# hahnyuan/PTQ4ViT

Hardware: AMD Instinct MI355X
Metric: calibration throughput (wrapped modules calibrated per second), ViT-B/224 W8A8, 32 calibration images (higher is better)
Workload: dtype int8

## Files before the change

### include/ptq4vit_hip_debug.h

```cpp
#ifndef PTQ4VIT_HIP_DEBUG_H
#define PTQ4VIT_HIP_DEBUG_H

#include <stdint.h>

#ifdef __cplusplus
extern "C" {
#endif

int p4v_debug_set_variant(int variant, int force_generic);
int p4v_debug_set_tuning(int key, int value);
int p4v_debug_topk_rows(const float* d_mass, int segs, int n, int k, int32_t* d_idx, void* stream);
int p4v_debug_pack_dual(const float* d_x, long rows, long cols, long cols_padded, int sos, int lo, int hi, int qmax,
                        const float* d_scale, float const_scale, int8_t* d_q1, int8_t* d_q2, void* stream);
int p4v_debug_pack_cands(const float* d_x, long rows, long cols, long rows_padded, long cols_padded, int layout, int lo, int hi,
                         const float* d_scales, int n_cands, const int* d_crange, const unsigned char* d_done, int live_max,
                         int general, int8_t* d_q, void* stream);
int p4v_debug_gather_im2col(int batch, int in_channels, int height, int width, int kernel_h, int kernel_w, int stride_h, int stride_w,
                            int pad_h, int pad_w, int dil_h, int dil_w, const float* d_x, const int32_t* d_idx, int k, float* d_dst,
                            void* stream);
int p4v_debug_prep_epi6(const float* d_o, const float* d_wt, const float* d_bias, long o_ss, long o_ts, int sr, int tr,
                        int bias_on_t, int wt_mode, int transposed, float* d_e, void* stream);

#ifdef __cplusplus
}
#endif
#endif
```

### ptq4vit_amd/_lib.py

```python
import ctypes as C
import os

_HERE = os.path.dirname(os.path.abspath(__file__))
LIB_PATH = os.environ.get("P4V_LIB") or os.path.join(_HERE, "csrc", "libptq4vit_hip.so")

METRICS = {
    "L1_norm": 0,
    "L2_norm": 1,
    "linear_weighted_L2_norm": 2,
    "square_weighted_L2_norm": 3,
    "hessian": 4,
    "cosine": 5,
}


class LinearDesc(C.Structure):
    _fields_ = [(n, C.c_int32) for n in (
        "batch", "tokens", "in_features", "out_features", "n_V", "n_H", "n_a", "w_bit", "a_bit", "metric",
        "eq_n", "search_round", "twin_postgelu", "init_layerwise", "has_bias", "reserved")]


class MatMulDesc(C.Structure):
    _fields_ = ([(n, C.c_int32) for n in ("batch", "heads", "M", "K", "N")] + [("_pad0", C.c_int32)] +
                [("a_stride", C.c_int64 * 4), ("b_stride", C.c_int64 * 4)] +
# ... 10 lines not shown
        "batch", "in_channels", "height", "width", "out_channels", "kernel_h", "kernel_w", "stride_h", "stride_w",
        "pad_h", "pad_w", "dil_h", "dil_w", "w_bit", "a_bit", "metric", "eq_n", "search_round", "channelwise",
        "init_layerwise", "has_bias", "reserved")]


class KernelStats(C.Structure):
    _fields_ = [("sweep_i8_ms", C.c_double), ("sweep_i8_launches", C.c_int64), ("sweep_i8_macs", C.c_double),
                ("sweep_f32_ms", C.c_double), ("sweep_f32_launches", C.c_int64), ("sweep_f32_macs", C.c_double),
                ("sweep_i8_alg_macs", C.c_double), ("sweep_f32_alg_macs", C.c_double),
                ("sweep6_ms", C.c_double), ("sweep6_launches", C.c_int64), ("sweep6_macs", C.c_double), ("sweep6_alg_macs", C.c_double),
                ("memo_hits", C.c_int64), ("memo_misses", C.c_int64),
                ("sweep7_ms", C.c_double), ("sweep7_launches", C.c_int64), ("sweep7_macs", C.c_double), ("sweep7_alg_macs", C.c_double),
                ("sweep7_twin_ms", C.c_double), ("sweep7_twin_launches", C.c_int64), ("event_overhead_ms", C.c_double)]


class LaunchRecord(C.Structure):
    _fields_ = [("kind", C.c_int32), ("stage", C.c_int32), ("grid_x", C.c_int32), ("grid_z", C.c_int32),
                ("ms", C.c_double), ("ops", C.c_double), ("alg_ops", C.c_double), ("alg_bytes", C.c_double)]


LAUNCH_KINDS = {0: "k_sweep<int8>", 1: "k_sweep<float>", 2: "k_sweep6", 3: "k_sweep7", 4: "k_sweep7 (twin)", 5: "k_sweep4/5", 6: "k_sweep9",
                7: "k_sweep8", 8: "k_sweep2g", 9: "k_sweep2", 11: "k_sos_split", 12: "k_bound", 13: "k_slice_b", 14: "k_slice_a", 15: "k_sweep_seg"}
LAUNCH_STAGES = {0: "full", 1: "A", 2: "B1", 3: "B2", 4: "A2"}


class PlaneDesc(C.Structure):
    _fields_ = [("rows", C.c_int64), ("cols", C.c_int64), ("cols_padded", C.c_int64), ("rows_per_scale", C.c_int64),
                ("mode", C.c_int32), ("lo", C.c_int32), ("hi", C.c_int32), ("qmax", C.c_int32),
                ("const_scale", C.c_float), ("reserved", C.c_int32)]


class ExportDesc(C.Structure):
    _fields_ = [("dims", C.c_int32 * 4), ("src_stride", C.c_int64 * 4),
                ("scale1_stride", C.c_int64 * 4), ("scale1_div", C.c_int32 * 4),
                ("scale2_stride", C.c_int64 * 4), ("scale2_div", C.c_int32 * 4),
                ("scale2_const", C.c_float),
                ("mode", C.c_int32), ("lo1", C.c_int32), ("hi1", C.c_int32), ("lo2", C.c_int32), ("hi2", C.c_int32),
                ("qmax", C.c_int32), ("reserved", C.c_int32)]


class GroupJob(C.Structure):
    _fields_ = [("kind", C.c_int32), ("status", C.c_int32), ("desc", C.c_void_p), ("inp", C.c_void_p * 5), ("mult", C.c_void_p),
                ("out", C.c_void_p * 3), ("workspace", C.c_void_p), ("workspace_bytes", C.c_size_t)]


JOB_LINEAR, JOB_MATMUL, JOB_CONV, JOB_MATMUL_BLOCKS = 0, 1, 2, 3
PLANE_SYM, PLANE_SOS_HI, PLANE_SOS_LO, PLANE_TWIN = 1, 2, 3, 4
EXPORT_SYM_I8, EXPORT_SYM_F32, EXPORT_GELU_U8, EXPORT_SOS_U8 = 0, 1, 2, 3


EXPORTS = [
    "p4v_version", "p4v_last_error",
    "p4v_linear_workspace_bytes", "p4v_linear_calibrate",
    "p4v_matmul_workspace_bytes", "p4v_matmul_calibrate",
    "p4v_matmul_blocks_workspace_bytes", "p4v_matmul_blocks_calibrate", "p4v_amax_init_matmul_blocks",
    "p4v_matmul_blocks_search", "p4v_matmul_blocks_quant_forward",
    "p4v_conv_workspace_bytes", "p4v_conv_calibrate",
    "p4v_calibrate_group", "p4v_launch_counters",
    "p4v_linear_quant_forward", "p4v_matmul_quant_forward",
    "p4v_amax_init_linear", "p4v_linear_search_w", "p4v_linear_search_a",
    "p4v_amax_init_matmul", "p4v_matmul_search_A", "p4v_sos_search_split", "p4v_matmul_search_B",
    "p4v_amax_init_conv", "p4v_conv_search_w_channelwise", "p4v_conv_search_w_layerwise", "p4v_conv_search_a",
    "p4v_score_argmax_gather",
    "p4v_quantize_i8", "p4v_pack_plane_i8", "p4v_fake_quant", "p4v_export_quantize", "p4v_multi_copy",
    "p4v_stats_enable", "p4v_stats_reset", "p4v_stats_get", "p4v_stats_launches", "p4v_prune_counters",
    "p4v_debug_set_variant", "p4v_debug_set_tuning", "p4v_debug_topk_rows", "p4v_debug_pack_dual", "p4v_debug_prep_epi6",
    "p4v_debug_pack_cands", "p4v_debug_gather_im2col",
]

_lib = None


def load():
    global _lib
    if _lib is not None:
        return _lib
    if not os.path.exists(LIB_PATH):
        raise RuntimeError(
            f"ptq4vit_amd: HIP extension {LIB_PATH} is missing -- build it with "
            "`python -c 'import __graft_entry__ as g; g.build()'` (hipcc --offload-arch=gfx950). "
            "There is no CPU fallback for the calibration path.")
    import torch
    lib = C.CDLL(LIB_PATH)
    vp, fp, ip = C.c_void_p, C.c_void_p, C.c_void_p
    lib.p4v_version.restype = C.c_int
    lib.p4v_last_error.restype = C.c_char_p
    lib.p4v_linear_workspace_bytes.restype = C.c_size_t
    lib.p4v_linear_workspace_bytes.argtypes = [C.POINTER(LinearDesc)]
    lib.p4v_linear_calibrate.restype = C.c_int
    lib.p4v_linear_calibrate.argtypes = [C.POINTER(LinearDesc), fp, fp, fp, fp, fp, fp, fp, fp, fp, ip, vp, C.c_size_t, vp]
# ... 38 lines not shown
        fn.restype = C.c_int
        fn.argtypes = args + tail
    lib.p4v_score_argmax_gather.restype = C.c_int
    lib.p4v_score_argmax_gather.argtypes = [fp, C.c_int32, C.c_int32, fp, fp, ip, vp]
    lib.p4v_quantize_i8.restype = C.c_int
    lib.p4v_quantize_i8.argtypes = [fp, C.c_int64, C.c_int64, C.c_int64, fp, C.c_int64, C.c_int32, C.c_int32, vp, vp]
    lib.p4v_fake_quant.restype = C.c_int
    lib.p4v_fake_quant.argtypes = [fp, C.c_int64, C.c_int64, fp, C.c_int64, C.c_int32, C.c_int32, fp, vp]
    lib.p4v_pack_plane_i8.restype = C.c_int
    lib.p4v_pack_plane_i8.argtypes = [C.POINTER(PlaneDesc), fp, fp, vp, vp]
    lib.p4v_export_quantize.restype = C.c_int
    lib.p4v_export_quantize.argtypes = [C.POINTER(ExportDesc), fp, fp, fp, vp, vp]
    lib.p4v_multi_copy.restype = C.c_int
    lib.p4v_multi_copy.argtypes = [vp, C.c_int32, C.c_int64, C.c_int64, vp]
    lib.p4v_debug_topk_rows.restype = C.c_int
    lib.p4v_debug_topk_rows.argtypes = [vp, C.c_int, C.c_int, C.c_int, vp, vp]
    lib.p4v_debug_pack_dual.restype = C.c_int
    lib.p4v_debug_pack_dual.argtypes = [fp, C.c_long, C.c_long, C.c_long, C.c_int, C.c_int, C.c_int, C.c_int, fp, C.c_float, vp, vp, vp]
    lib.p4v_debug_pack_cands.restype = C.c_int
    lib.p4v_debug_pack_cands.argtypes = [fp, C.c_long, C.c_long, C.c_long, C.c_long, C.c_int, C.c_int, C.c_int, fp, C.c_int, vp, vp,
                                         C.c_int, C.c_int, vp, vp]
    lib.p4v_debug_gather_im2col.restype = C.c_int
    lib.p4v_debug_gather_im2col.argtypes = [C.c_int] * 12 + [fp, ip, C.c_int, fp, vp]
    lib.p4v_debug_prep_epi6.restype = C.c_int
    lib.p4v_debug_prep_epi6.argtypes = [fp, fp, fp, C.c_long, C.c_long, C.c_int, C.c_int, C.c_int, C.c_int, C.c_int, fp, vp]
    lib.p4v_debug_set_variant.restype = C.c_int
    lib.p4v_debug_set_variant.argtypes = [C.c_int, C.c_int]
    lib.p4v_debug_set_tuning.restype = C.c_int
    lib.p4v_debug_set_tuning.argtypes = [C.c_int, C.c_int]
    lib.p4v_stats_enable.restype = C.c_int
    lib.p4v_stats_enable.argtypes = [C.c_int]
    lib.p4v_stats_reset.restype = C.c_int
    lib.p4v_stats_get.restype = C.c_int
    lib.p4v_stats_get.argtypes = [C.POINTER(KernelStats)]
    lib.p4v_stats_launches.restype = C.c_int
    lib.p4v_stats_launches.argtypes = [C.POINTER(LaunchRecord), C.c_int64, C.POINTER(C.c_int64)]
    lib.p4v_prune_counters.restype = C.c_int
    lib.p4v_prune_counters.argtypes = [C.POINTER(C.c_int64), C.c_int]
    lib.p4v_launch_counters.restype = C.c_int
    lib.p4v_launch_counters.argtypes = [C.POINTER(C.c_int64), C.c_int]
    lib.p4v_calibrate_group.restype = C.c_int
    lib.p4v_calibrate_group.argtypes = [C.POINTER(GroupJob), C.c_int32, vp, vp]
    _lib = lib
    return lib


# ... 17 lines not shown
```

### ptq4vit_amd/csrc/p4v_api.hip

```cpp
#include <hip/hip_runtime.h>

#include <algorithm>
#include <atomic>
#include <climits>
#include <cstdarg>
#include <cstdio>
#include <condition_variable>
#include <cstring>
#include <deque>
#include <functional>
#include <thread>
#include <mutex>
#include <string>
#include <unordered_map>
#include <type_traits>
#include <vector>

#include "../../include/ptq4vit_hip.h"
#include "../../include/ptq4vit_hip_debug.h"
#include "p4v_kernels.h"

using namespace p4v;

namespace {
// ... 43 lines not shown
        return (dry || top > cap) ? nullptr : base + cap - top;
    }
    bool ok() const { return dry || off + top <= cap; }
};

struct StatRec { hipEvent_t a, b; int kind; double macs, alg; int stage, gx, gz; double ms, bytes; };
thread_local double g_alg_bytes = 0;
thread_local double g_alg_macs_cand = 0;
thread_local double g_exec_frac = 1.0;
thread_local bool g_stat_on = false;
thread_local std::vector<StatRec> g_stat_recs;
thread_local std::vector<StatRec> g_stat_done;
thread_local int g_stage = 0;
thread_local p4v_kernel_stats g_stats = {};
thread_local long g_memo_hits = 0, g_memo_misses = 0;
std::atomic<long long> g_prune_cnt[4];
constexpr int VARIANT_KEPT = 1 | 2 | 4 | 2048 | 32768 | 65536 | 131072 | 524288 | 1048576 | 2097152 | 4194304 | 8388608 | 134217728;
std::atomic<int> g_variant_word{0};
#define g_variant (g_variant_word.load(std::memory_order_relaxed) & 0x3fffffff)
#define g_force_v1 ((g_variant_word.load(std::memory_order_relaxed) >> 30) & 1)
std::atomic<int> g_tune[16];
enum { TUNE_CG6 = 0, TUNE_CG2 = 1, TUNE_CG2G = 2, TUNE_CG7 = 3, TUNE_PRINT = 4, TUNE_ORDER7 = 5, TUNE_P6 = 6, TUNE_PLANE_GIB = 7, TUNE_EPI6W = 8,
       TUNE_LOOSE_PCT = 9, TUNE_SLICE_DIV = 10, TUNE_SLICE_SMALL = 11, TUNE_B1_PATH = 12, TUNE_TIER2 = 13, TUNE_TIER2_DIV = 14, TUNE_LOOSE_ROWS = 15 };
inline bool tune_b1_removed(int v) { return v == 1 || v == 2 || v == 3 || v == 5 || v == 6 || v == 8 || v == 10 || v == 12; }
inline int tune(int k) { return g_tune[k].load(std::memory_order_relaxed); }

struct Group;
struct Ctx {
    hipStream_t st;
    Arena ws;
    bool dry;
    Group* grp = nullptr;
    int slot = 0;
    int par = 1;
};

struct StatInfo { int kind; double macs, alg; int stage, gx, gz; double bytes; };
struct QOp;
struct KernelDesc {
    hipError_t (*one)(const QOp&, hipStream_t);
    hipError_t (*many)(const QOp* const*, int, hipStream_t);
    int cap;
};
constexpr int QOP_PARAM_BYTES = 480;
struct QOp {
    enum Type : int { KERNEL, FILL, D2H, H2D, COPY2D, WAIT };
    int type = KERNEL;
// ... 73 lines not shown
    int n = 0;
    std::mutex mu;
    std::condition_variable cv;
    std::vector<std::deque<QOp>> q;
    std::vector<int> state;
    int blocked = 0;
    unsigned long gen = 0;
    int status = 0;
    std::string err;
    std::vector<int*> mirrors;
    bool stat_on = false;
    std::vector<StatRec>* stat_recs = nullptr;
    long n_ops = 0, n_launches = 0, n_rounds = 0;
    hipEvent_t inputs_ready = nullptr;
    bool waited = false;
    int last_par[16] = {};
    int issue_kernels(std::vector<const QOp*>& ops);
    int issue_round();
    int sync(int slot);
    void finish(int slot);
};

std::atomic<long long> g_launch_cnt[4];
int enqueue_now(hipStream_t st, const QOp& op, bool timed, std::vector<StatRec>* recs) {
    g_launch_cnt[1].fetch_add(1, std::memory_order_relaxed);
    StatRec rec{};
    if (timed) {
        HIPCHK(hipEventCreate(&rec.a));
        HIPCHK(hipEventCreate(&rec.b));
        HIPCHK(hipEventRecord(rec.a, st));
    }
    HIPCHK(op.kd->one(op, st));
    if (timed) {
        HIPCHK(hipEventRecord(rec.b, st));
        rec.kind = op.si.kind; rec.macs = op.si.macs; rec.alg = op.si.alg; rec.stage = op.si.stage; rec.gx = op.si.gx; rec.gz = op.si.gz; rec.bytes = op.si.bytes;
        recs->push_back(rec);
    }
    return 0;
}
int issue_plain(hipStream_t st, const QOp& op) {
    switch (op.type) {
        case QOp::FILL: HIPCHK(hipMemsetAsync(op.dst, op.value, op.bytes, st)); break;
        case QOp::D2H: HIPCHK(hipMemcpyAsync(op.dst, op.src, op.bytes, hipMemcpyDeviceToHost, st)); break;
        case QOp::H2D: HIPCHK(hipMemcpyAsync(op.dst, op.payload.data(), op.bytes, hipMemcpyHostToDevice, st)); break;
        case QOp::COPY2D: HIPCHK(hipMemcpy2DAsync(op.dst, op.dpitch, op.src, op.spitch, op.width, op.height, hipMemcpyDeviceToDevice, st)); break;
        default: break;
// ... 491 lines not shown
    cgroups = std::max(cgroups, cdiv(nc, per_max));
    const int per = cdiv(nc, cgroups);
    const size_t lds = (size_t)SW7_NS * SW7_STAGE + (size_t)per * 192 + 256;
    Sweep7Params q = p;
    q.cgroups = cgroups;
    dim3 grid(p.rtiles * p.ctiles * cgroups, 1, 1);
    const StatInfo si = stat_info(twin ? 4 : 3, (double)p.rtiles * 256 * (double)p.ctiles * 256 * (double)p.ldk * nc, g_alg_macs_cand * nc,
                                  (int)grid.x, (int)grid.z, g_alg_bytes);
    const StatInfo* sp = &si;
    return twin == 2 ? launch_sweep7_epi<2>(c, q, epi, grid, lds, sp) : twin ? launch_sweep7_epi<1>(c, q, epi, grid, lds, sp) : launch_sweep7_epi<0>(c, q, epi, grid, lds, sp);
}

int launch_sweep(Ctx& c, const SweepParams& p, bool i8, bool twin, int epi, bool fast = false, int cgroups = 1) {
    if (c.dry) return 0;
    const int kind = (fast && p.bound) ? 12 : (fast && p.halves > 0) ? 6 : (fast && sweep8_ok(p, twin, epi)) ? 7 :
                     (fast && epi != EPI_COS && sweep2g_ok(p)) ? 8 : fast ? 9 : i8 ? 0 : 1;
    const double kelems = (double)p.ldk / (i8 ? 1 : 4);
    const StatInfo si = stat_info(kind, (double)p.mtiles * SW_BM * (double)p.ntiles * SW_BN * kelems * p.Z * (p.c1 - p.c0) * (twin ? 2 : 1),
                                  g_alg_macs_cand * (p.c1 - p.c0),
                                  (fast && p.bound) ? p.mtiles * p.ntiles * 2 : (fast && p.halves > 0) ? p.halves : p.mtiles * p.ntiles, cgroups, g_alg_bytes);
    const StatInfo* sp = &si;
    if (fast && p.bound) {
        const dim3 grid(p.mtiles * p.ntiles * 2), block(256);
        P4V_EPI4(epi, return enqueue(c, KERN_T(SweepParams, k_bound, E), grid, block, 0, p, sp))
    }
    if (fast && p.halves > 0) return p.a_cs == 0 ? launch_sweep9_epi<true>(c, p, epi, cgroups, sp) : launch_sweep9_epi<false>(c, p, epi, cgroups, sp);
    if (fast && sweep8_ok(p, twin, epi)) return p.a_cs == 0 ? launch_sweep8_epi<true>(c, p, epi, cgroups, sp) : launch_sweep8_epi<false>(c, p, epi, cgroups, sp);
    if (fast && epi != EPI_COS && sweep2g_ok(p)) return twin ? launch_sweep2g_epi<true>(c, p, epi, cgroups, sp) : launch_sweep2g_epi<false>(c, p, epi, cgroups, sp);
    if (fast) return twin ? launch_sweep2_epi<true>(c, p, epi, cgroups, sp) : launch_sweep2_epi<false>(c, p, epi, cgroups, sp);
    if (i8) return twin ? launch_sweep_epi<int8_t, true>(c, p, epi, cgroups, sp) : launch_sweep_epi<int8_t, false>(c, p, epi, cgroups, sp);
    return twin ? launch_sweep_epi<float, true>(c, p, epi, cgroups, sp) : launch_sweep_epi<float, false>(c, p, epi, cgroups, sp);
}

int launch_finish(Ctx& c, const FinishParams& p) {
    return enqueue(c, KERN(FinishParams, k_finish), dim3(p.C, p.nj), dim3(256), 0, p);
}

int launch_finish_cos(Ctx& c, const FinishCosParams& p) {
    const int gy = p.j_mode == 3 ? cdiv(p.S, 256) : p.nj;
    return enqueue(c, KERN(FinishCosParams, k_finish_cos), dim3(p.C, gy), dim3(p.j_mode == 3 ? 256 : 1024), 0, p);
}

int launch_select(Ctx& c, const SelectParams& p_) {
    if (c.dry) return 0;
    SelectParams p = p_;
    attach_mirror(p);
    return enqueue(c, KERN(SelectParams, k_select), dim3(p.nj), dim3(128), 0, p);
// ... 496 lines not shown
        sp.ldk = Kp * esz; sp.ktiles = sp.ldk / SW_BKB;
        sp.S1 = S1; sp.S2 = S2; sp.s_cs = ps.s_cs; sp.sb_mode = ps.sb_mode; sp.sb_div = std::max(1, ps.sb_div);
        sp.bias = ps.bias; sp.bias_axis = ps.bias_axis; sp.bias_zs = ps.bias_zs;
        sp.O = ps.O; sp.Wt = ps.G ? ps.G : ps.O; sp.wt_mode = ps.wt_mode;
        sp.o_zs = ps.o_zs; sp.o_bs = ps.o_bs; sp.o_ms = ps.o_ms; sp.o_nbs = ps.o_nbs; sp.o_ns = ps.o_ns;
        sp.o_inner = ps.o_inner > 0 ? ps.o_inner : INT_MAX;
        sp.o_ninner = ps.o_ninner > 0 ? ps.o_ninner : INT_MAX;
        sp.M = ps.Mrows; sp.N = ps.Ncols; sp.Z = ps.Z; sp.c0 = c0; sp.c1 = c0 + nc; sp.crange = ps.crange;
        sp.crange_blk = rblk_z; sp.cb_div = std::max(1, ps.j_div);
        sp.part = part; sp.p_cs = p_cs; sp.p_zs = p_zs; sp.Np = NpP;
        sp.mtiles = Mp / SW_BM; sp.ntiles = Np / SW_BN;
        sp.dbg = g_variant & 3;
        sp.store = ps.store_out;
        int cgroups = 1;
        if (!fast && !fast_cos) {
            const long wgs = (long)sp.mtiles * sp.ntiles * ps.Z;
            cgroups = choose_cgroups(wgs, nc, sp.ktiles, cu_slots(c, 512, ps.i8 ? 0 : 1), 20.0, ps.i8 ? 1.6 : 2.6);
        }
        if (fast || fast_cos) {
            const long wgs = (long)sp.mtiles * sp.ntiles * ps.Z;
            cgroups = choose_cgroups(wgs, nc, sp.ktiles, cu_slots(c, ps.twin ? 256 : 512, 9), ps.twin ? 40.0 : 25.0, ps.twin ? 0.45 : 0.40);
        }
        sp.bound = bound ? 1 : 0;
        if (bound) sp.dbg = tune(TUNE_B1_PATH) >= 16 ? (tune(TUNE_B1_PATH) >> 4) : 0;
        if (bound) { sp.A = rowbuf; sp.B = colbuf; sp.a_cs = sp.b_cs = 0; }
        if (fast && !bound && !ps.store_out && (ps.j_mode == 0 || ps.j_mode == 2)) {
            const int h9 = sweep9_halves(sp, ps.twin, ps.epi);
            if (h9 > 0 && (long)h9 * SW9_NW <= p_zs) {
                sp.halves = h9;
                sp.rows_p_stream = sp.a_cs == 0 ? Np : Mp;
                sp.p_zs = (long)h9 * SW9_NW; sp.p_cs = sp.p_zs * ps.Z;
                nine_halves = h9;
                cgroups = choose_cgroups((long)h9 * ps.Z, nc, 1, cu_slots(c, SW9_NW == 4 ? 512 : 256, 6), 12.0, 0.9);
            }
        }
        if (fast && !ps.store_out) {
            if (const int t_ = tune(sweep2g_ok(sp) ? TUNE_CG2G : TUNE_CG2); t_ > 0) cgroups = std::max(1, std::min(nc, t_));
            if (tune(TUNE_PRINT) > 0) fprintf(stderr, "[p4v] sweep2%s tiles %d x %d z %d ktiles %d cand %d twin %d -> cgroups %d\n", sweep2g_ok(sp) ? "g" : "", sp.mtiles, sp.ntiles, ps.Z, sp.ktiles, nc, (int)ps.twin, cgroups);
        }
        CHK(launch_sweep(c, sp, ps.i8, ps.twin, ps.epi, fast || fast_cos, cgroups));
    }
    g_exec_frac = 1.0;
    if (ps.store_out) { c.ws.off = mark; return 0; }
    auto with_marks = [&](FinishParams& fp) {
        if (ps.crange && pc && pc->done) { fp.mark_done = pc->done; fp.mark_n = ps.eq_n; }
        fp.crange_blk = rblk ? rblk : rblk_z;
    };
// ... 1986 lines not shown
    p.src = d_x; p.conv = 1; p.ic = in_channels; p.H = height; p.W = width; p.kh = kernel_h; p.kw = kernel_w;
    p.sh = stride_h; p.sw = stride_w; p.ph = pad_h; p.pw = pad_w; p.dh = dil_h; p.dw = dil_w;
    p.fw = fw; p.L = fh * fw;
    p.Z = 1; p.s_z = 0; p.R = batch * fh * fw; p.K = in_channels * kernel_h * kernel_w; p.nblk_r = 1; p.nblk_k = 1;
    p.mode = PACK_RAW;
    Ctx c{(hipStream_t)stream, Arena(nullptr, 0), false};
    const long total = (long)k * p.K;
    return enqueue(c, KERN(GatherIm2colParams, k_gather_im2col), dim3((unsigned)std::min<long>(cdiv(total, 256), 256L * 16)), dim3(256), 0,
                   GatherIm2colParams{p, d_idx, k, d_dst});
}

int p4v_debug_prep_epi6(const float* d_o, const float* d_wt, const float* d_bias, long o_ss, long o_ts, int sr, int tr,
                        int bias_on_t, int wt_mode, int transposed, float* d_e, void* stream) {
    if (!d_o || !d_bias || !d_e || (wt_mode == 1 && !d_wt) || sr <= 0 || tr <= 0 || wt_mode < 0 || wt_mode > 4)
        return fail(P4V_ERR_INVALID, "p4v_debug_prep_epi6: bad argument");
    PrepEpi6Params pe{};
    pe.O = d_o; pe.Wt = d_wt ? d_wt : d_o; pe.bias = d_bias; pe.o_ss = o_ss; pe.o_ts = o_ts; pe.SR = sr; pe.TR = tr;
    pe.bias_on_t = bias_on_t ? 1 : 0; pe.wt_mode = wt_mode; pe.transposed = transposed ? 1 : 0;
    pe.stiles = cdiv(sr, 256); pe.ttiles = cdiv(tr, 64); pe.E = d_e;
    Ctx c{(hipStream_t)stream, Arena(nullptr, 0), false};
    return enqueue(c, KERN(PrepEpi6Params, k_prep_epi6), dim3((unsigned)std::min<long>((long)pe.stiles * pe.ttiles, 256L * 32)), dim3(256), 0, pe);
}

int p4v_pack_plane_i8(const p4v_plane_desc* d, const float* d_x, const float* d_scales, int8_t* d_q, void* stream) {
    if (!d || !d_x || !d_q || d->rows <= 0 || d->cols <= 0 || d->cols_padded % 64 || d->cols_padded < d->cols)
        return fail(P4V_ERR_INVALID, "p4v_pack_plane_i8: bad argument");
    if (d->mode != P4V_PLANE_SYM && d->mode != P4V_PLANE_SOS_HI && d->mode != P4V_PLANE_SOS_LO && d->mode != P4V_PLANE_TWIN)
        return fail(P4V_ERR_INVALID, "p4v_pack_plane_i8: unknown mode %d", d->mode);
    if (d->mode == P4V_PLANE_TWIN && (d->lo > 0 || d->hi < 0 || !(d->const_scale > 0.0f)))
        return fail(P4V_ERR_INVALID, "p4v_pack_plane_i8: the merged twin plane needs lo <= 0 <= hi and const_scale > 0");
    if (d->mode != P4V_PLANE_SYM && !d_scales) return fail(P4V_ERR_INVALID, "p4v_pack_plane_i8: split-of-softmax planes need d_scales = &split");
    if (d->mode == P4V_PLANE_SYM && d_scales && d->rows_per_scale <= 0) return fail(P4V_ERR_INVALID, "p4v_pack_plane_i8: rows_per_scale");
    if (d->lo < -128 || d->hi > 127 || d->qmax < 2 || d->qmax > 128) return fail(P4V_ERR_INVALID, "p4v_pack_plane_i8: grid wider than int8");
    Ctx c{(hipStream_t)stream, Arena(nullptr, 0), false};
    cvt_bias(c);
    PackParams p = pack2d(d_x, d->rows, d->cols, d->cols);
    p.Rp = (int)d->rows; p.Kp = (int)d->cols_padded; p.dst = d_q; p.C = 1;
    p.scales = d_scales; p.sc_cs = 0; p.neg_scale = d->const_scale;
    p.lo = d->lo; p.hi = d->hi; p.qm1 = (float)(d->qmax - 1);
    if (d->mode == P4V_PLANE_SYM) {
        p.mode = PACK_SYM;
        if (d_scales) { p.blk_mode = 1; p.blk_div = (int)d->rows_per_scale; p.nblk_r = cdiv(d->rows, d->rows_per_scale); p.nblk_k = 1; }
    } else if (d->mode == P4V_PLANE_TWIN) {
        p.mode = PACK_TWIN_I8;
    } else {
        p.mode = d->mode == P4V_PLANE_SOS_HI ? PACK_SOS_HI : PACK_SOS_LO;
// ... 32 lines not shown
```

### ptq4vit_amd/csrc/p4v_kernels.h

```cpp
#pragma once
#include <hip/hip_runtime.h>
#include <stdint.h>
#include <type_traits>

namespace p4v {

typedef int v4i __attribute__((ext_vector_type(4)));
typedef int v16i __attribute__((ext_vector_type(16)));
typedef float v4f __attribute__((ext_vector_type(4)));
typedef float v16f __attribute__((ext_vector_type(16)));
typedef float v2f __attribute__((ext_vector_type(2)));

#ifndef P4V_GROUP_KERNARG
#define P4V_GROUP_KERNARG (4096 - 256)
#endif
template <typename P> struct GroupArgs {
    static constexpr int CAP_RAW = (P4V_GROUP_KERNARG - 16) / (int)(sizeof(P) + 16);
    static constexpr int CAP = CAP_RAW > 64 ? 64 : CAP_RAW;
    int n;
    unsigned off[CAP + 1];
    unsigned gx[CAP], gy[CAP], gz[CAP];
    P p[CAP];
};
#define P4V_BIDX uint3{blockIdx.x, blockIdx.y, blockIdx.z}
// ... 1172 lines not shown
    };
    if (total > 2) wait_vmcnt<NPL * 2>(); else if (total > 1) wait_vmcnt<NPL>(); else wait_vmcnt<0>();
    __builtin_amdgcn_s_barrier();
    read_fr(fa, std::integral_constant<int, 0>{});
    for (int it = 0; it < total; it += SW2_NS) {
        tile(it, std::integral_constant<int, 0>{}, fa, fb);
        if (it + 1 < total) tile(it + 1, std::integral_constant<int, 1>{}, fb, fa);
        if (it + 2 < total) tile(it + 2, std::integral_constant<int, 2>{}, fa, fb);
        if (it + 3 < total) tile(it + 3, std::integral_constant<int, 3>{}, fb, fa);
    }
#undef P4V_DSR
    __syncthreads();
    if constexpr (STORES || EPI == EPI_COS) return;
    for (int i = tid; i < (c_hi - c_lo) * 8; i += 512) {
        const int cc = c_lo + i / 8, wv = i % 8;
        p.part[(long)cc * p.p_cs + (long)z * p.p_zs + (long)(mt * 2 + (wv >> 2)) * p.Np + nt * 4 + (wv & 3)] = res[i];
    }
}
template <bool TWIN, int EPI>
__global__ __launch_bounds__(512, 2) void k_sweep2(SweepParams p) { k_sweep2_body<TWIN, EPI>(p, P4V_BIDX, P4V_GDIM); }
template <bool TWIN, int EPI>
__global__ __launch_bounds__(512, 2) void k_sweep2_g(GroupArgs<SweepParams> a) { P4V_GROUP_ENTER(a); k_sweep2_body<TWIN, EPI>(a.p[m_], vb_, vg_); }

template <int EPI>
__device__ __forceinline__ void k_bound_body(const SweepParams& p, const uint3 blockIdx, const uint3 gridDim) {
    const int tid = threadIdx.x, lane = tid & 63;
    const int wid = __builtin_amdgcn_readfirstlane(tid >> 6);
    const int g = lane >> 5, l31 = lane & 31;
    const int ntiles = p.ntiles * 2;
    const int nwg = p.mtiles * ntiles;
    const int t = xcd_remap(blockIdx.x, nwg);
    constexpr int GM = 4;
    const int per_group = GM * ntiles;
    const int first_m = (t / per_group) * GM;
    const int gsz = min(p.mtiles - first_m, GM);
    const int mt = first_m + (t % per_group) % gsz, nt = (t % per_group) / gsz;
    int c = p.c0;
    if (p.crange) {
        const int a = __builtin_amdgcn_readfirstlane(p.crange[0]), b = __builtin_amdgcn_readfirstlane(p.crange[1]);
        if (a >= b) return;
        c = max(c, a);
        if (c >= b) return;
    }
    if (c >= p.c1) return;
    const int wr = wid >> 1, wc = wid & 1;
    const int m0 = mt * 128 + wr * 64, n0 = nt * 64 + wc * 32;
    float* slot = p.part + (long)c * p.p_cs + (long)(mt * 2 + wr) * p.Np + nt * 2 + wc;
    if (m0 >= p.M || n0 >= p.N) {
        if (lane == 63) slot[0] = 0.0f;
        return;
    }
    const char* sA = (const char*)p.A + (long)(m0 >> 6) * p.ktiles * 4096;
    const char* sB = (const char*)p.B + (long)(n0 >> 6) * p.ktiles * 4096 + ((n0 >> 5) & 1) * 2048;
    const unsigned vo = (unsigned)lane * 16u;
    v16i acc[2];
#pragma unroll
    for (int i = 0; i < 2; ++i)
#pragma unroll
        for (int r = 0; r < 16; ++r) acc[i][r] = 0;
    struct Fr { v4i a[2][2], b[2]; };
#define P4V_BLD(dst, voff, sbase, off) asm volatile("global_load_dwordx4 %0, %1, %2 offset:%3" : "=v"(dst) : "v"(voff), "s"(sbase), "n"(off) : "memory")
    auto load = [&](Fr& f) __attribute__((always_inline)) {
        P4V_BLD(f.a[0][0], vo, sA, 0); P4V_BLD(f.a[0][1], vo, sA, 1024);
        P4V_BLD(f.b[0], vo, sB, 0); P4V_BLD(f.b[1], vo, sB, 1024);
        P4V_BLD(f.a[1][0], vo, sA, 2048); P4V_BLD(f.a[1][1], vo, sA, 3072);
        sA += 4096; sB += 4096;
    };
    auto mma = [&](Fr& f) __attribute__((always_inline)) {
        asm volatile("" : "+v"(f.a[0][0]), "+v"(f.a[0][1]), "+v"(f.a[1][0]), "+v"(f.a[1][1]), "+v"(f.b[0]), "+v"(f.b[1]) :: "memory");
#pragma unroll
        for (int h = 0; h < 2; ++h)
#pragma unroll
            for (int i = 0; i < 2; ++i) acc[i] = __builtin_amdgcn_mfma_i32_32x32x32_i8(f.a[i][h], f.b[h], acc[i], 0, 0, 0);
    };
    Fr f0, f1, f2;
    const int ktiles = p.ktiles;
    constexpr int LD = 6;
    load(f0);
    if (ktiles > 1) load(f1);
    auto step = [&](int kt, Fr& cur, Fr& refill) __attribute__((always_inline)) {
        const int ahead = min(ktiles - 1 - kt, 2);
        if (kt + 2 < ktiles) load(refill);
        if (ahead >= 2) wait_vmcnt<2 * LD>(); else if (ahead == 1) wait_vmcnt<LD>(); else wait_vmcnt<0>();
        mma(cur);
    };
    for (int kt = 0; kt < ((p.dbg & 1) ? 1 : ktiles); kt += 3) {
        step(kt, f0, f2);
        if (kt + 1 < ktiles) step(kt + 1, f1, f0);
        if (kt + 2 < ktiles) step(kt + 2, f2, f1);
    }
#undef P4V_BLD
    const int n = n0 + l31;
    const bool ncol_ok = n < p.N;
    const int nc = min(n, p.N - 1);
    const float bias_n = (p.bias && ncol_ok) ? p.bias[nc] : 0.0f;
    const int sb = p.sb_mode == 1 ? min(nc / p.sb_div, p.s_cs - 1) : 0;
    const float s1 = p.S1 ? p.S1[(long)c * p.s_cs + sb] : 1.0f;
    const float* On = p.O + (long)nc * p.o_ns;
    const float* Wn = p.Wt + (long)nc * p.o_ns;
    float sum = 0.0f;
#pragma unroll
    for (int i = 0; i < 2; ++i) {
        float u[16], w[16];
#pragma unroll
        for (int r = 0; r < 16; ++r) {
            const int mc = (p.dbg & 2) ? 0 : min(m0 + i * 32 + (r & 3) + 8 * (r >> 2) + 4 * g, p.M - 1);
            u[r] = On[(long)mc * p.o_ms];
            if (EPI == EPI_SQ_W || EPI == EPI_W_SQ) w[r] = Wn[(long)mc * p.o_ms];
        }
#pragma unroll
        for (int r = 0; r < 16; ++r) {
            const int m = m0 + i * 32 + (r & 3) + 8 * (r >> 2) + 4 * g;
            const bool ok = ncol_ok && m < p.M;
            const float o = u[r];
            float wv = 1.0f;
            if (EPI == EPI_SQ_W) wv = w[r]; else if (EPI == EPI_W_SQ) wv = fabsf(w[r]);
            const float d = (o - bias_n) - (float)acc[i][r] * s1;
            float term;
            if (EPI == EPI_SQ_W) { const float t2 = wv * d; term = t2 * t2; }
            else if (EPI == EPI_SQ) term = d * d;
            else if (EPI == EPI_ABS) term = fabsf(d);
            else term = (wv * d) * d;
            sum += ok ? term : 0.0f;
        }
        asm volatile("" ::: "memory");
    }
    sum = wave_sum_dpp(sum);
    if (lane == 63) slot[0] = sum;
}
template <int EPI>
__global__ __launch_bounds__(256, 4) void k_bound(SweepParams p) { k_bound_body<EPI>(p, P4V_BIDX, P4V_GDIM); }
template <int EPI>
__global__ __launch_bounds__(256, 4) void k_bound_g(GroupArgs<SweepParams> a) { P4V_GROUP_ENTER(a); k_bound_body<EPI>(a.p[m_], vb_, vg_); }

static constexpr int SW8_NS = 8;

#ifndef P4V_SW8_DBG
#define P4V_SW8_DBG 0
#endif
template <bool ROWS_FIXED, int EPI, bool SKIP>
__device__ __forceinline__ void k_sweep8_body(const SweepParams& p, const uint3 blockIdx, const uint3 gridDim) {
    extern __shared__ __attribute__((aligned(16))) char smem[];
    float* res = reinterpret_cast<float*>(smem + SW8_NS * SW2_TILE);

    const int tid = threadIdx.x, lane = tid & 63;
    const int wid = __builtin_amdgcn_readfirstlane(tid >> 6);
    const int g = lane >> 5, l31 = lane & 31;

    const int nwg = p.mtiles * p.ntiles;
// ... 2722 lines not shown
```

### ptq4vit_amd/engine.py

```python
import ctypes as C

import torch

from . import _lib

_workspace = {}
_mult_cache = {}


def _require_cuda(t, what):
    if not t.is_cuda:
        raise RuntimeError(f"ptq4vit_amd: {what} must live on the GPU (got {t.device}); the calibration path has no CPU fallback")


def device_of(*tensors):
    for t in tensors:
        if t is not None and t.is_cuda:
            return t.device
    if not torch.cuda.is_available():
        raise RuntimeError("ptq4vit_amd: no GPU visible -- the HIP calibration engine needs an MI355X (no CPU fallback)")
    return torch.device("cuda", torch.cuda.current_device())


def to_dev(t, dev):
# ... 655 lines not shown
    b, ic, H, W = x.shape
    (kh, kw), (sh, sw), (ph, pw), (dh, dw) = kernel_size, stride, padding, dilation
    fh, fw = (H + 2 * ph - dh * (kh - 1) - 1) // sh + 1, (W + 2 * pw - dw * (kw - 1) - 1) // sw + 1
    if fh > 0 and fw > 0:
        assert idx.numel() > 0 and int(idx.min()) >= 0 and int(idx.max()) < b * fh * fw, "row index outside the im2col matrix"
    out = torch.full((idx.numel(), ic * kh * kw), float("nan"), dtype=torch.float32, device=x.device)
    with torch.cuda.device(x.device):
        rc = _lib.load().p4v_debug_gather_im2col(b, ic, H, W, kh, kw, sh, sw, ph, pw, dh, dw, ptr(x), ptr(idx), idx.numel(), ptr(out),
                                                 stream_ptr(x.device))
    _lib.check(rc, "p4v_debug_gather_im2col")
    return out


def debug_prep_epi6(o, wt, bias, *, o_ss, o_ts, sr, tr, bias_on_t, wt_mode, transposed):
    n = -(-sr // 256) * -(-tr // 64) * 256 * 64 * 2
    e = torch.full((n,), float("nan"), dtype=torch.float32, device=o.device)
    with torch.cuda.device(o.device):
        rc = _lib.load().p4v_debug_prep_epi6(ptr(o), ptr(wt) if wt is not None else None, ptr(bias), int(o_ss), int(o_ts),
                                             int(sr), int(tr), int(bias_on_t), int(wt_mode), int(transposed), ptr(e),
                                             stream_ptr(o.device))
    _lib.check(rc, "p4v_debug_prep_epi6")
    return e

def stats_reset():
    _lib.load().p4v_stats_reset()


def stats_get():
    s = _lib.KernelStats()
    _lib.check(_lib.load().p4v_stats_get(C.byref(s)), "p4v_stats_get")
    return {k: getattr(s, k) for k, _ in _lib.KernelStats._fields_}


def prune_counters(reset=False):
    out = (C.c_int64 * 4)()
    _lib.check(_lib.load().p4v_prune_counters(out, int(bool(reset))), "p4v_prune_counters")
    return dict(zip(("staged", "staged_no_survivors", "kept_full_sweep", "not_eligible"), (int(v) for v in out)))


def stats_launches():
    lib = _lib.load()
    n = C.c_int64(0)
    _lib.check(lib.p4v_stats_launches(None, 0, C.byref(n)), "p4v_stats_launches")
    buf = (_lib.LaunchRecord * max(1, n.value))()
    _lib.check(lib.p4v_stats_launches(buf, n.value, C.byref(n)), "p4v_stats_launches")
    return [{"kernel": _lib.LAUNCH_KINDS.get(r.kind, str(r.kind)), "stage": _lib.LAUNCH_STAGES.get(r.stage, str(r.stage)),
# ... 3 lines not shown
```

Baseline: 668.2.

## Stage k_bound operand tiles through LDS with a 3-slot async pipeline

```diff
diff --git a/include/ptq4vit_hip_debug.h b/include/ptq4vit_hip_debug.h
--- a/include/ptq4vit_hip_debug.h
+++ b/include/ptq4vit_hip_debug.h
@@ -21,6 +21,15 @@
 int p4v_debug_prep_epi6(const float* d_o, const float* d_wt, const float* d_bias, long o_ss, long o_ts, int sr, int tr,
                         int bias_on_t, int wt_mode, int transposed, float* d_e, void* stream);
 
+typedef struct p4v_bound_member {
+    const float* x; const float* w; const float* bias; const float* out; const float* wt;
+    const float* scale_x; const float* scale_w;
+    int32_t M, K, N, n_blocks;
+    float* totals;
+} p4v_bound_member;
+int p4v_debug_bound_scores(const p4v_bound_member* members, int n_members, int metric, int a_bit, int w_bit, int grouped,
+                           void* d_workspace, size_t workspace_bytes, void* stream);
+
 #ifdef __cplusplus
 }
 #endif
diff --git a/ptq4vit_amd/_lib.py b/ptq4vit_amd/_lib.py
--- a/ptq4vit_amd/_lib.py
+++ b/ptq4vit_amd/_lib.py
@@ -56,6 +56,11 @@
 LAUNCH_KINDS = {0: "k_sweep<int8>", 1: "k_sweep<float>", 2: "k_sweep6", 3: "k_sweep7", 4: "k_sweep7 (twin)", 5: "k_sweep4/5", 6: "k_sweep9",
                 7: "k_sweep8", 8: "k_sweep2g", 9: "k_sweep2", 11: "k_sos_split", 12: "k_bound", 13: "k_slice_b", 14: "k_slice_a", 15: "k_sweep_seg"}
 LAUNCH_STAGES = {0: "full", 1: "A", 2: "B1", 3: "B2", 4: "A2"}
+
+
+class BoundMember(C.Structure):
+    _fields_ = ([(n, C.c_void_p) for n in ("x", "w", "bias", "out", "wt", "scale_x", "scale_w")] +
+                [(n, C.c_int32) for n in ("M", "K", "N", "n_blocks")] + [("totals", C.c_void_p)])
 
 
 class PlaneDesc(C.Structure):
@@ -99,7 +104,7 @@
     "p4v_quantize_i8", "p4v_pack_plane_i8", "p4v_fake_quant", "p4v_export_quantize", "p4v_multi_copy",
     "p4v_stats_enable", "p4v_stats_reset", "p4v_stats_get", "p4v_stats_launches", "p4v_prune_counters",
     "p4v_debug_set_variant", "p4v_debug_set_tuning", "p4v_debug_topk_rows", "p4v_debug_pack_dual", "p4v_debug_prep_epi6",
-    "p4v_debug_pack_cands", "p4v_debug_gather_im2col",
+    "p4v_debug_pack_cands", "p4v_debug_gather_im2col", "p4v_debug_bound_scores",
 ]
 
 _lib = None
@@ -184,6 +189,8 @@
                                          C.c_int, C.c_int, vp, vp]
     lib.p4v_debug_gather_im2col.restype = C.c_int
     lib.p4v_debug_gather_im2col.argtypes = [C.c_int] * 12 + [fp, ip, C.c_int, fp, vp]
+    lib.p4v_debug_bound_scores.restype = C.c_int
+    lib.p4v_debug_bound_scores.argtypes = [C.POINTER(BoundMember), C.c_int, C.c_int, C.c_int, C.c_int, C.c_int, vp, C.c_size_t, vp]
     lib.p4v_debug_prep_epi6.restype = C.c_int
     lib.p4v_debug_prep_epi6.argtypes = [fp, fp, fp, C.c_long, C.c_long, C.c_int, C.c_int, C.c_int, C.c_int, C.c_int, fp, vp]
     lib.p4v_debug_set_variant.restype = C.c_int
diff --git a/ptq4vit_amd/csrc/p4v_api.hip b/ptq4vit_amd/csrc/p4v_api.hip
--- a/ptq4vit_amd/csrc/p4v_api.hip
+++ b/ptq4vit_amd/csrc/p4v_api.hip
@@ -89,7 +89,7 @@
 std::atomic<int> g_tune[16];
 enum { TUNE_CG6 = 0, TUNE_CG2 = 1, TUNE_CG2G = 2, TUNE_CG7 = 3, TUNE_PRINT = 4, TUNE_ORDER7 = 5, TUNE_P6 = 6, TUNE_PLANE_GIB = 7, TUNE_EPI6W = 8,
        TUNE_LOOSE_PCT = 9, TUNE_SLICE_DIV = 10, TUNE_SLICE_SMALL = 11, TUNE_B1_PATH = 12, TUNE_TIER2 = 13, TUNE_TIER2_DIV = 14, TUNE_LOOSE_ROWS = 15 };
-inline bool tune_b1_removed(int v) { return v == 1 || v == 2 || v == 3 || v == 5 || v == 6 || v == 8 || v == 10 || v == 12; }
+inline bool tune_b1_removed(int v) { return v == 1 || v == 2 || v == 3 || v == 5 || v == 6 || v == 8 || v == 10 || v == 12 || v >= 16; }
 inline int tune(int k) { return g_tune[k].load(std::memory_order_relaxed); }
 
 struct Group;
@@ -209,6 +209,7 @@
 };
 
 std::atomic<long long> g_launch_cnt[4];
+std::atomic<long long> g_bound_launches{0};
 int enqueue_now(hipStream_t st, const QOp& op, bool timed, std::vector<StatRec>* recs) {
     g_launch_cnt[1].fetch_add(1, std::memory_order_relaxed);
     StatRec rec{};
@@ -746,7 +747,8 @@
     const StatInfo* sp = &si;
     if (fast && p.bound) {
         const dim3 grid(p.mtiles * p.ntiles * 2), block(256);
-        P4V_EPI4(epi, return enqueue(c, KERN_T(SweepParams, k_bound, E), grid, block, 0, p, sp))
+        g_bound_launches.fetch_add(1, std::memory_order_relaxed);
+        P4V_EPI4(epi, return enqueue(c, KERN_T(SweepParams, k_bound, E), grid, block, BND_LDS, p, sp))
     }
     if (fast && p.halves > 0) return p.a_cs == 0 ? launch_sweep9_epi<true>(c, p, epi, cgroups, sp) : launch_sweep9_epi<false>(c, p, epi, cgroups, sp);
     if (fast && sweep8_ok(p, twin, epi)) return p.a_cs == 0 ? launch_sweep8_epi<true>(c, p, epi, cgroups, sp) : launch_sweep8_epi<false>(c, p, epi, cgroups, sp);
@@ -1289,7 +1291,7 @@
             cgroups = choose_cgroups(wgs, nc, sp.ktiles, cu_slots(c, ps.twin ? 256 : 512, 9), ps.twin ? 40.0 : 25.0, ps.twin ? 0.45 : 0.40);
         }
         sp.bound = bound ? 1 : 0;
-        if (bound) sp.dbg = tune(TUNE_B1_PATH) >= 16 ? (tune(TUNE_B1_PATH) >> 4) : 0;
+        if (bound) sp.dbg = 0;
         if (bound) { sp.A = rowbuf; sp.B = colbuf; sp.a_cs = sp.b_cs = 0; }
         if (fast && !bound && !ps.store_out && (ps.j_mode == 0 || ps.j_mode == 2)) {
             const int h9 = sweep9_halves(sp, ps.twin, ps.epi);
@@ -3322,6 +3324,63 @@
     return enqueue(c, KERN(PrepEpi6Params, k_prep_epi6), dim3((unsigned)std::min<long>((long)pe.stiles * pe.ttiles, 256L * 32)), dim3(256), 0, pe);
 }
 
+int p4v_debug_bound_scores(const p4v_bound_member* members, int n_members, int metric, int a_bit, int w_bit, int grouped,
+                           void* d_workspace, size_t workspace_bytes, void* stream) {
+    if (!members || n_members <= 0 || n_members > 16 || !d_workspace || a_bit < 2 || a_bit > 8 || w_bit < 2 || w_bit > 8)
+        return fail(P4V_ERR_INVALID, "p4v_debug_bound_scores: bad argument");
+    int epi, wt_mode;
+    metric_epi(metric, &epi, &wt_mode);
+    if (epi == EPI_COS) return fail(P4V_ERR_UNSUPPORTED, "p4v_debug_bound_scores: k_bound has no cosine epilogue");
+    const int aq = 1 << (a_bit - 1), wq = 1 << (w_bit - 1);
+    const hipStream_t st = (hipStream_t)stream;
+    cvt_probe(st);
+    auto member_pass = [&](const p4v_bound_member& m, Pass& ps) -> int {
+        if (!m.x || !m.w || !m.out || !m.scale_x || !m.scale_w || !m.totals || m.M <= 0 || m.K <= 0 || m.N <= 0 || m.n_blocks <= 0 ||
+            m.N % m.n_blocks || (m.n_blocks > 1 && (m.N / m.n_blocks) % 32) || (wt_mode == 1 && !m.wt))
+            return fail(P4V_ERR_INVALID, "p4v_debug_bound_scores: bad member (score blocks must be whole 32-column groups)");
+        ps = Pass{};
+        ps.i8 = true; ps.twin = false; ps.epi = epi; ps.wt_mode = wt_mode; ps.eq_n = 1; ps.K = m.K;
+        ps.Z = 1; ps.Mrows = m.M; ps.Ncols = m.N;
+        ps.row.present = true; ps.row.expanded = false;
+        ps.row.pk = pack2d(m.x, m.M, m.K, m.K);
+        ps.row.pk.scales = m.scale_x; ps.row.pk.sc_cs = 0; ps.row.pk.lo = -aq; ps.row.pk.hi = aq - 1;
+        ps.col.present = true; ps.col.expanded = true;
+        ps.col.pk = pack2d(m.w, m.N, m.K, m.K);
+        ps.col.pk.blk_mode = 1; ps.col.pk.blk_div = m.N / m.n_blocks; ps.col.pk.nblk_r = m.n_blocks; ps.col.pk.nblk_k = 1;
+        ps.col.pk.scales = m.scale_w; ps.col.pk.sc_cs = m.n_blocks; ps.col.pk.lo = -wq; ps.col.pk.hi = wq - 1;
+        ps.use_s1 = true; ps.s_cs = m.n_blocks; ps.sb_mode = 1; ps.sb_div = m.N / m.n_blocks;
+        ps.s1 = ScaleParams{m.scale_x, 0, 0, 0.f, m.scale_w, m.n_blocks, 1, 0.f, 0, 0, nullptr};
+        ps.bias = m.bias; ps.bias_axis = 0; ps.bias_zs = 0;
+        ps.O = m.out; ps.G = wt_mode == 1 ? m.wt : nullptr; ps.o_ms = m.N; ps.o_ns = 1; ps.o_inner = INT_MAX;
+        ps.j_mode = 1; ps.j_div = m.N / m.n_blocks; ps.nj = m.n_blocks; ps.norm = -1.0;
+        ps.cands = m.scale_w; ps.cand_cs = m.n_blocks; ps.cand_js = 1;
+        ps.scores_keep = m.totals; ps.no_select = true; ps.bound_kernel = true;
+        return 0;
+    };
+    const size_t share = (workspace_bytes / (size_t)n_members) & ~(size_t)255;
+    std::vector<Pass> passes(n_members);
+    for (int i = 0; i < n_members; ++i) CHK(member_pass(members[i], passes[i]));
+    const long long before = g_bound_launches.load(std::memory_order_relaxed);
+    if (!grouped || n_members == 1) {
+        for (int i = 0; i < n_members; ++i) {
+            Ctx c{st, Arena((char*)d_workspace + share * i, share), false};
+            CHK(run_pass(c, passes[i]));
+        }
+    } else {
+        Group g;
+        g.st = st; g.n = n_members;
+        g.q.resize(n_members); g.state.assign(n_members, 0); g.mirrors.assign(n_members, nullptr);
+        for (int i = 0; i < n_members; ++i) {
+            Ctx c{st, Arena((char*)d_workspace + share * i, share), false, &g, i, 1};
+            CHK(run_pass(c, passes[i]));
+        }
+        CHK(g.issue_round());
+    }
+    if (g_bound_launches.load(std::memory_order_relaxed) == before)
+        return fail(P4V_ERR_UNSUPPORTED, "p4v_debug_bound_scores: the pass did not qualify for k_bound");
+    return 0;
+}
+
 int p4v_pack_plane_i8(const p4v_plane_desc* d, const float* d_x, const float* d_scales, int8_t* d_q, void* stream) {
     if (!d || !d_x || !d_q || d->rows <= 0 || d->cols <= 0 || d->cols_padded % 64 || d->cols_padded < d->cols)
         return fail(P4V_ERR_INVALID, "p4v_pack_plane_i8: bad argument");
diff --git a/ptq4vit_amd/csrc/p4v_kernels.h b/ptq4vit_amd/csrc/p4v_kernels.h
--- a/ptq4vit_amd/csrc/p4v_kernels.h
+++ b/ptq4vit_amd/csrc/p4v_kernels.h
@@ -1218,8 +1218,12 @@
 template <bool TWIN, int EPI>
 __global__ __launch_bounds__(512, 2) void k_sweep2_g(GroupArgs<SweepParams> a) { P4V_GROUP_ENTER(a); k_sweep2_body<TWIN, EPI>(a.p[m_], vb_, vg_); }
 
+static constexpr int BND_NS = 3;
+static constexpr int BND_SLOT = 12 * 1024;
+static constexpr int BND_LDS = BND_NS * BND_SLOT;
 template <int EPI>
 __device__ __forceinline__ void k_bound_body(const SweepParams& p, const uint3 blockIdx, const uint3 gridDim) {
+    extern __shared__ __attribute__((aligned(16))) char smem[];
     const int tid = threadIdx.x, lane = tid & 63;
     const int wid = __builtin_amdgcn_readfirstlane(tid >> 6);
     const int g = lane >> 5, l31 = lane & 31;
@@ -1242,68 +1246,92 @@
     const int wr = wid >> 1, wc = wid & 1;
     const int m0 = mt * 128 + wr * 64, n0 = nt * 64 + wc * 32;
     float* slot = p.part + (long)c * p.p_cs + (long)(mt * 2 + wr) * p.Np + nt * 2 + wc;
-    if (m0 >= p.M || n0 >= p.N) {
+    if (mt * 128 >= p.M || nt * 64 >= p.N) {
         if (lane == 63) slot[0] = 0.0f;
         return;
     }
-    const char* sA = (const char*)p.A + (long)(m0 >> 6) * p.ktiles * 4096;
-    const char* sB = (const char*)p.B + (long)(n0 >> 6) * p.ktiles * 4096 + ((n0 >> 5) & 1) * 2048;
-    const unsigned vo = (unsigned)lane * 16u;
-    v16i acc[2];
-#pragma unroll
-    for (int i = 0; i < 2; ++i)
-#pragma unroll
-        for (int r = 0; r < 16; ++r) acc[i][r] = 0;
-    struct Fr { v4i a[2][2], b[2]; };
-#define P4V_BLD(dst, voff, sbase, off) asm volatile("global_load_dwordx4 %0, %1, %2 offset:%3" : "=v"(dst) : "v"(voff), "s"(sbase), "n"(off) : "memory")
-    auto load = [&](Fr& f) __attribute__((always_inline)) {
-        P4V_BLD(f.a[0][0], vo, sA, 0); P4V_BLD(f.a[0][1], vo, sA, 1024);
-        P4V_BLD(f.b[0], vo, sB, 0); P4V_BLD(f.b[1], vo, sB, 1024);
-        P4V_BLD(f.a[1][0], vo, sA, 2048); P4V_BLD(f.a[1][1], vo, sA, 3072);
-        sA += 4096; sB += 4096;
-    };
-    auto mma = [&](Fr& f) __attribute__((always_inline)) {
-        asm volatile("" : "+v"(f.a[0][0]), "+v"(f.a[0][1]), "+v"(f.a[1][0]), "+v"(f.a[1][1]), "+v"(f.b[0]), "+v"(f.b[1]) :: "memory");
-#pragma unroll
-        for (int h = 0; h < 2; ++h)
-#pragma unroll
-            for (int i = 0; i < 2; ++i) acc[i] = __builtin_amdgcn_mfma_i32_32x32x32_i8(f.a[i][h], f.b[h], acc[i], 0, 0, 0);
-    };
-    Fr f0, f1, f2;
+    const bool act = m0 < p.M && n0 < p.N;
     const int ktiles = p.ktiles;
-    constexpr int LD = 6;
-    load(f0);
-    if (ktiles > 1) load(f1);
-    auto step = [&](int kt, Fr& cur, Fr& refill) __attribute__((always_inline)) {
-        const int ahead = min(ktiles - 1 - kt, 2);
-        if (kt + 2 < ktiles) load(refill);
-        if (ahead >= 2) wait_vmcnt<2 * LD>(); else if (ahead == 1) wait_vmcnt<LD>(); else wait_vmcnt<0>();
-        mma(cur);
-    };
-    for (int kt = 0; kt < ((p.dbg & 1) ? 1 : ktiles); kt += 3) {
-        step(kt, f0, f2);
-        if (kt + 1 < ktiles) step(kt + 1, f1, f0);
-        if (kt + 2 < ktiles) step(kt + 2, f2, f1);
-    }
-#undef P4V_BLD
+
+    constexpr bool HAS_W = EPI == EPI_SQ_W || EPI == EPI_W_SQ;
     const int n = n0 + l31;
     const bool ncol_ok = n < p.N;
     const int nc = min(n, p.N - 1);
-    const float bias_n = (p.bias && ncol_ok) ? p.bias[nc] : 0.0f;
-    const int sb = p.sb_mode == 1 ? min(nc / p.sb_div, p.s_cs - 1) : 0;
-    const float s1 = p.S1 ? p.S1[(long)c * p.s_cs + sb] : 1.0f;
     const float* On = p.O + (long)nc * p.o_ns;
     const float* Wn = p.Wt + (long)nc * p.o_ns;
+    auto ld_epi = [&](int i, float (&u)[16], float (&w)[16]) __attribute__((always_inline)) {
+#pragma unroll
+        for (int r = 0; r < 16; ++r) {
+            const int mc = min(m0 + i * 32 + (r & 3) + 8 * (r >> 2) + 4 * g, p.M - 1);
+            u[r] = On[(long)mc * p.o_ms];
+            if (HAS_W) w[r] = Wn[(long)mc * p.o_ms];
+        }
+    };
+    float u0[16], w0[16], u1[16], w1[16];
+    float bias_n = 0.0f, s1 = 1.0f;
+    if (act) {
+        ld_epi(0, u0, w0);
+        bias_n = (p.bias && ncol_ok) ? p.bias[nc] : 0.0f;
+        const int sb = p.sb_mode == 1 ? min(nc / p.sb_div, p.s_cs - 1) : 0;
+        s1 = p.S1 ? p.S1[(long)c * p.s_cs + sb] : 1.0f;
+    }
+
+    constexpr int NP = 3;
+    const char* src[NP];
+#pragma unroll
+    for (int q = 0; q < NP; ++q) {
+        const int j = wid * NP + q;
+        src[q] = (j < 8 ? (const char*)p.A + (long)(mt * 2 + (j >> 2)) * ktiles * 4096 + (j & 3) * 1024
+                        : (const char*)p.B + (long)nt * ktiles * 4096 + (j - 8) * 1024) + lane * 16;
+    }
+    char* const dst0 = smem + wid * (NP * 1024);
+    auto issue = [&](int stage) __attribute__((always_inline)) {
+#pragma unroll
+        for (int q = 0; q < NP; ++q) {
+            glds16(src[q], dst0 + stage * BND_SLOT + q * 1024);
+            src[q] += 4096;
+        }
+    };
+    v16i acc[2];
+#pragma unroll
+    for (int i = 0; i < 2; ++i)
+#pragma unroll
+        for (int r = 0; r < 16; ++r) acc[i][r] = 0;
+    const unsigned lds0 = (unsigned)(unsigned long long)(__attribute__((address_space(3))) char*)smem;
+    const unsigned aA = lds0 + wr * 4096 + lane * 16, aB = lds0 + 8192 + wc * 2048 + lane * 16;
+#define P4V_DSR(dst, addr, off) asm volatile("ds_read_b128 %0, %1 offset:%2" : "=v"(dst) : "v"(addr), "n"(off))
+    auto step = [&](int kt, auto st_c) __attribute__((always_inline)) {
+        constexpr int ST = decltype(st_c)::value;
+        if (kt + 1 < ktiles) wait_vmcnt<NP>(); else wait_vmcnt<0>();
+        __builtin_amdgcn_s_barrier();
+        if (kt + 2 < ktiles) issue((ST + 2) % BND_NS);
+        if (!act) return;
+        constexpr int SO = ST * BND_SLOT;
+        v4i a00, a01, a10, a11, b0, b1;
+        P4V_DSR(a00, aA, SO); P4V_DSR(b0, aB, SO); P4V_DSR(a10, aA, SO + 2048);
+        P4V_DSR(a01, aA, SO + 1024); P4V_DSR(b1, aB, SO + 1024); P4V_DSR(a11, aA, SO + 3072);
+        __builtin_amdgcn_s_waitcnt(0xC07F);
+        asm volatile("" : "+v"(a00), "+v"(a01), "+v"(a10), "+v"(a11), "+v"(b0), "+v"(b1) :: "memory");
+        acc[0] = __builtin_amdgcn_mfma_i32_32x32x32_i8(a00, b0, acc[0], 0, 0, 0);
+        acc[1] = __builtin_amdgcn_mfma_i32_32x32x32_i8(a10, b0, acc[1], 0, 0, 0);
+        acc[0] = __builtin_amdgcn_mfma_i32_32x32x32_i8(a01, b1, acc[0], 0, 0, 0);
+        acc[1] = __builtin_amdgcn_mfma_i32_32x32x32_i8(a11, b1, acc[1], 0, 0, 0);
+    };
+    issue(0);
+    if (ktiles > 1) issue(1);
+    for (int kt = 0; kt < ktiles; kt += BND_NS) {
+        step(kt, std::integral_constant<int, 0>{});
+        if (kt + 1 < ktiles) step(kt + 1, std::integral_constant<int, 1>{});
+        if (kt + 2 < ktiles) step(kt + 2, std::integral_constant<int, 2>{});
+    }
+#undef P4V_DSR
+    if (!act) {
+        if (lane == 63) slot[0] = 0.0f;
+        return;
+    }
+    ld_epi(1, u1, w1);
     float sum = 0.0f;
-#pragma unroll
-    for (int i = 0; i < 2; ++i) {
-        float u[16], w[16];
-#pragma unroll
-        for (int r = 0; r < 16; ++r) {
-            const int mc = (p.dbg & 2) ? 0 : min(m0 + i * 32 + (r & 3) + 8 * (r >> 2) + 4 * g, p.M - 1);
-            u[r] = On[(long)mc * p.o_ms];
-            if (EPI == EPI_SQ_W || EPI == EPI_W_SQ) w[r] = Wn[(long)mc * p.o_ms];
-        }
+    auto block = [&](int i, const float (&u)[16], const float (&w)[16]) __attribute__((always_inline)) {
 #pragma unroll
         for (int r = 0; r < 16; ++r) {
             const int m = m0 + i * 32 + (r & 3) + 8 * (r >> 2) + 4 * g;
@@ -1319,8 +1347,9 @@
             else term = (wv * d) * d;
             sum += ok ? term : 0.0f;
         }
-        asm volatile("" ::: "memory");
-    }
+    };
+    block(0, u0, w0);
+    block(1, u1, w1);
     sum = wave_sum_dpp(sum);
     if (lane == 63) slot[0] = sum;
 }
diff --git a/ptq4vit_amd/engine.py b/ptq4vit_amd/engine.py
--- a/ptq4vit_amd/engine.py
+++ b/ptq4vit_amd/engine.py
@@ -701,6 +701,34 @@
     _lib.check(rc, "p4v_debug_prep_epi6")
     return e
 
+
+def debug_bound_scores(members, *, metric, a_bit=8, w_bit=8, grouped=False):
+    dev = members[0]["x"].device
+    keep, arr = [], (_lib.BoundMember * len(members))()
+    outs = []
+    need = 0
+    for i, m in enumerate(members):
+        t = {k: (v.contiguous().float() if v is not None else None) for k, v in m.items() if k in ("x", "w", "bias", "out", "wt", "scale_x", "scale_w")}
+        M, K = t["x"].shape
+        N = t["w"].shape[0]
+        nb = t["scale_w"].numel()
+        assert t["w"].shape[1] == K and t["out"].shape == (M, N) and t["scale_x"].numel() == 1
+        tot = torch.full((nb,), float("nan"), dtype=torch.float32, device=dev)
+        keep.append(t); outs.append(tot)
+        for k in ("x", "w", "bias", "out", "wt", "scale_x", "scale_w"):
+            setattr(arr[i], k, ptr(t[k]) if t.get(k) is not None else None)
+        arr[i].M, arr[i].K, arr[i].N, arr[i].n_blocks, arr[i].totals = M, K, N, nb, ptr(tot)
+        Kp = (K + 63) // 64 * 64
+        need = max(need, ((M + 127) // 128 * 128 + (N + 127) // 128 * 128) * Kp + 8 * ((M + 127) // 128) * 2 * (N + 127) // 128 * 128 + (1 << 20))
+    ws = torch.empty(need * len(members), dtype=torch.uint8, device=dev)
+    with torch.cuda.device(dev):
+        rc = _lib.load().p4v_debug_bound_scores(arr, len(members), _lib.METRICS[metric], int(a_bit), int(w_bit), int(bool(grouped)),
+                                                ptr(ws), ws.numel(), stream_ptr(dev))
+        _lib.check(rc, "p4v_debug_bound_scores")
+        torch.cuda.synchronize(dev)
+    return outs
+
+
 def stats_reset():
     _lib.load().p4v_stats_reset()
 
```

Result: no change. 674.2 (median of 6 runs) (+0.9%).
